# Fannovel16/ComfyUI-Frame-Interpolation

Hardware: AMD Instinct MI355X
Metric: interpolated frames/sec/GPU @1080p RIFE4.7 2x (higher is better)
Workload: dtype f32; 1 GPU; RIFE 4.7 2x, 1080x1920 synthetic frame-pair stream, 32 pairs/step/GPU resident in HBM (BASELINE.json configs[1]; SURVEY 8d config 2 clip: 33 frames torch.manual_seed(0) torch.rand); seeded random-init weights; new_frame_collective=none, launch=one process, one GPU

## Files before the change

comfyui-frame-interpolation_amd/csrc/rife_net.hip:

```cpp
#include <cmath>
#include <cstring>

#include "../../include/vfi_hip.h"
#include "../../include/vfi_hip_test.h"
#include "rife_ops.h"

using namespace vfi;

namespace {

struct DevBuf {
    float* p = nullptr;
    size_t n = 0;
    bool view = false;
    int ensure(size_t count) {
        if (count <= n) return 0;
        if (p && !view) (void)hipFree(p);
        p = nullptr;
        n = 0;
        view = false;
        VFI_CHECK_HIP(hipMalloc((void**)&p, count * sizeof(float)));
        n = count;
        return 0;
    }
// ... 33 lines not shown
    DevBuf w, ww, bias, beta;
    DevBuf bias3;
    int Cout3_p = 0;
    int Cin = 0, Cin_p = 0, Cout = 0, Cout_p = 0;
    bool folded = false;
};

const int kBlockC[5] = {192, 128, 96, 64, 32};
constexpr int kMaxBlocks = 5;

}

struct vfi_rife {
    ConvLayer conv00[kMaxBlocks], conv01[kMaxBlocks], res[kMaxBlocks][8], last[kMaxBlocks];
    DevBuf enc_w0, enc_b0, enc_w1, enc_b1;
    int arch = 47, NF = 1, CM = 16, CF = 4, n_mid = 0, nblocks = 4, NX = 0;
    bool enc_act = false;
    int last_out() const { return NX ? 52 : 24; }
    int tplanes() const { return NX ? 4 : 2; }
    DevBuf FEAT;
    ConvLayer enc_mid[2];
    DevBuf E2;
    int block_in(int i) const { return i == 0 ? 7 + 8 * NF : 12 + 8 * NF + NX; }
    int CX(int i) const { return round_up(block_in(i), 8); }
    int H = 0, W = 0, Hp = 0, Wp = 0, max_batch = 0, n_slots = 0;
    int scales[kMaxBlocks] = {8, 4, 2, 1, 1};
    int up[kMaxBlocks] = {1, 1, 1, 1, 1};
    DevBuf Ppool, E, F, F2, M, X, A0, A1, A2, T;
    DevBuf S0pool;
    std::vector<unsigned char> s0_valid;
    size_t stage0_stride() const { return (size_t)(Hp / 8) * (Wp / 8) * 8; }
    bool fused_pack() const { return n_mid == 0 && CM == 16 && CF == 4 && !enc_act && NF == 1; }
    DevBuf X1, T1;
    DevBuf Fdbg[kMaxBlocks], Xdbg[kMaxBlocks];
    bool keep = false;
    int last_B = 0;
    float* arena = nullptr;
    size_t arena_n = 0;
    std::vector<WeightView> views;
    int device = 0;
    size_t pack_stride() const { return (size_t)Hp * Wp * 4 * (1 + NF); }
};

static int bind_arena(vfi_rife* net, const std::vector<WeightView>& views, size_t n, const float* host) {
    VFI_CHECK_HIP(hipGetDevice(&net->device));
    VFI_CHECK_HIP(hipMalloc((void**)&net->arena, n * sizeof(float)));
    net->arena_n = n;
    if (host) VFI_CHECK_HIP(hipMemcpy(net->arena, host, n * sizeof(float), hipMemcpyHostToDevice));
    net->views = views;
    for (const WeightView& v : views) {
        DevBuf* b = (DevBuf*)((char*)net + v.delta);
        b->p = net->arena + v.off;
        b->n = v.count;
        b->view = true;
    }
    return 0;
}

static int make_conv3x3(ConvLayer& L, const float* w, const float* b, const float* beta, int Cout, int Cin,
                        int Cin_p, bool wino = false) {
    L.Cin = Cin;
    L.Cin_p = Cin_p;
    L.Cout = Cout;
    L.Cout_p = round_up(Cout, 32);
    std::vector<float> wp, bp;
    std::vector<float> wfold;
// ... 163 lines not shown

int vfi_rife_weights(vfi_rife_t* net, float** arena_dev, int64_t* count) {
    VFI_REQUIRE(net && net->arena && arena_dev && count, "vfi_rife_weights: null argument / no weights");
    *arena_dev = net->arena;
    *count = (int64_t)net->arena_n;
    return 0;
}

void vfi_rife_destroy(vfi_rife_t* net) {
    if (!net) return;
    for (int b = 0; b < kMaxBlocks; ++b) {
        for (ConvLayer* L : {&net->conv00[b], &net->conv01[b], &net->last[b]}) {
            L->w.release();
            L->ww.release();
            L->bias.release();
            L->beta.release();
        }
        for (int i = 0; i < 8; ++i) {
            net->res[b][i].w.release();
            net->res[b][i].ww.release();
            net->res[b][i].bias.release();
            net->res[b][i].beta.release();
        }
        net->Fdbg[b].release();
        net->Xdbg[b].release();
    }
    for (ConvLayer& L : net->enc_mid) {
        L.w.release();
        L.ww.release();
        L.bias.release();
    }
    net->E2.release();
    for (DevBuf* d : {&net->enc_w0, &net->enc_b0, &net->enc_w1, &net->enc_b1, &net->Ppool, &net->E, &net->F, &net->F2, &net->M,
                      &net->X, &net->A0, &net->A1, &net->A2, &net->T, &net->X1, &net->T1, &net->FEAT, &net->S0pool})
        d->release();
    if (net->arena) (void)hipFree(net->arena);
    delete net;
}

int vfi_rife_configure(vfi_rife_t* net, int H, int W, int max_batch, int n_slots, float scale_factor) {
    VFI_REQUIRE(net, "vfi_rife_configure: null handle");
    VFI_REQUIRE(H > 0 && W > 0 && max_batch >= 1 && max_batch <= kMaxTasks && n_slots >= 2,
                "vfi_rife_configure: bad arguments H=%d W=%d max_batch=%d (1..%d) n_slots=%d", H, W, max_batch,
                kMaxTasks, n_slots);
    const int NB = net->nblocks;
    const float base4[kMaxBlocks] = {8.f, 4.f, 2.f, 1.f, 1.f}, base5[kMaxBlocks] = {16.f, 8.f, 4.f, 2.f, 1.f};
    const float* base = NB == 5 ? base5 : base4;
    int sc[kMaxBlocks] = {1, 1, 1, 1, 1}, up[kMaxBlocks] = {1, 1, 1, 1, 1};
    for (int i = 0; i < NB; ++i) {
        const float s = base[i] / scale_factor;
        if (s >= 1.f) {
            sc[i] = (int)s;
            up[i] = 1;
            VFI_REQUIRE((float)sc[i] == s && (sc[i] == 1 || sc[i] % 2 == 0),
                        "vfi_rife_configure: scale_factor %g gives block scale %g (supported scale_factor: 0.25, 0.5, 1, 2, 4)",
                        scale_factor, s);
        } else {
            sc[i] = 1;
            up[i] = (int)(1.f / s);
            VFI_REQUIRE((up[i] == 2 || up[i] == 4) && 1.f / (float)up[i] == s && i > 0,
                        "vfi_rife_configure: scale_factor %g gives block scale %g (supported scale_factor: 0.25, 0.5, 1, 2, 4)",
                        scale_factor, s);
        }
    }
    const int Hp = round_up(H, 64), Wp = round_up(W, 64);
    for (int i = 0; i < NB; ++i) {
        VFI_REQUIRE(Hp % (4 * sc[i]) == 0 && Wp % (4 * sc[i]) == 0,
                    "vfi_rife_configure: padded size %dx%d not divisible by 4*scale %d (the reference fails here too, "
                    "SURVEY.md App. C6)", Hp, Wp, sc[i]);
        VFI_REQUIRE((double)Hp * Wp * up[i] * up[i] * net->CX(i) < 2147483647.0,
                    "vfi_rife_configure: %dx%d is too large for scale_factor %g (block input above 2^31 elements)", H, W,
                    scale_factor);
    }
    net->H = H;
    net->W = W;
    net->Hp = Hp;
    net->Wp = Wp;
    net->max_batch = max_batch;
    net->n_slots = n_slots;
    memcpy(net->scales, sc, sizeof(sc));
    memcpy(net->up, up, sizeof(up));
    const size_t full = (size_t)Hp * Wp, B = max_batch;
    size_t x = 0, a0 = 0, a1 = 0, t = 0;
    bool any_up = false;
    for (int i = 0; i < NB; ++i) {
        any_up = any_up || up[i] > 1;
        const size_t px = full / ((size_t)sc[i] * sc[i]) * ((size_t)up[i] * up[i]);
        const size_t cx = net->CX(i);
        x = std::max(x, px * cx);
        a0 = std::max(a0, px / 4 * (kBlockC[i] / 2));
        a1 = std::max(a1, px / 16 * kBlockC[i]);
        t = std::max(t, px * 4 * net->tplanes());
    }
    if (net->Ppool.ensure(net->pack_stride() * n_slots) || net->E.ensure(full / 4 * net->CM) ||
        (net->n_mid && net->E2.ensure(full / 4 * net->CM)) || net->F.ensure(B * full * 4) || net->F2.ensure(B * full * 4) ||
        net->M.ensure(B * full) || net->X.ensure(B * x) || net->A0.ensure(B * a0) || net->A1.ensure(B * a1) ||
        net->A2.ensure(B * a1) || net->T.ensure(B * t))
        return -1;
    if (any_up && (net->X1.ensure(B * full * net->CX(1)) || net->T1.ensure(B * full * 4 * net->tplanes()))) return -1;
    if (net->NX && net->FEAT.ensure(B * full * 8)) return -1;
    net->s0_valid.assign(n_slots, 0);
    if (net->fused_pack() && net->S0pool.ensure(net->stage0_stride() * n_slots)) return -1;
    return 0;
}

static void fill_args(ConvArgs& a, const ConvLayer& L, const float* in, int in_cs, float* out, int out_cs, int N,
                      int Hin, int Win, int stride) {
    memset(&a, 0, sizeof(a));
    a.in = in;
    a.w = L.w.p;
    a.bias = L.bias.p;
    a.out = out;
    a.N = N;
    a.Hin = Hin;
    a.Win = Win;
    a.in_cs = in_cs;
    a.Hout = Hin / stride;
    a.Wout = Win / stride;
    a.out_cs = out_cs;
    a.Cin_p = L.Cin_p;
    a.cin_live = L.Cin;
    a.Cout_p = L.Cout_p;
    a.Cout = L.Cout;
}

static int load_frame_impl(vfi_rife_t* net, int slot, const float* f32, const unsigned char* u8, int C, void* stream) {
    VFI_REQUIRE(net && net->Hp > 0, "vfi_rife_load_frame: network not configured");
    VFI_REQUIRE(slot >= 0 && slot < net->n_slots && C >= 3, "vfi_rife_load_frame: bad slot %d / channels %d", slot, C);
    hipStream_t st = (hipStream_t)stream;
    float* P = net->Ppool.p + (size_t)slot * net->pack_stride();
    const int Hp = net->Hp, Wp = net->Wp;
    const bool fuse_encode = option(kOptFuseEncode) != 0;
    net->s0_valid[slot] = 0;
// ... 63 lines not shown
    return 0;
}

int vfi_f32_to_u8(const float* in_dev, uint8_t* out_dev, int64_t n, void* stream) {
    VFI_REQUIRE(in_dev && out_dev && n >= 0 && ((uintptr_t)in_dev & 15) == 0 && ((uintptr_t)out_dev & 3) == 0,
                "vfi_f32_to_u8: bad arguments (in 16-byte, out 4-byte aligned)");
    return n ? f32_to_u8_launch(in_dev, out_dev, (long)n, (hipStream_t)stream) : 0;
}

int vfi_rife_interpolate(vfi_rife_t* net, int B, const int* slot0, const int* slot1, const float* timestep,
                         float* out_dev, void* stream) {
    VFI_REQUIRE(net && net->Hp > 0, "vfi_rife_interpolate: network not configured");
    VFI_REQUIRE(B >= 1 && B <= net->max_batch, "vfi_rife_interpolate: batch %d outside 1..%d", B, net->max_batch);
    hipStream_t st = (hipStream_t)stream;
    RifeTasks tasks;
    memset(&tasks, 0, sizeof(tasks));
    for (int b = 0; b < B; ++b) {
        VFI_REQUIRE(slot0[b] >= 0 && slot0[b] < net->n_slots && slot1[b] >= 0 && slot1[b] < net->n_slots,
                    "vfi_rife_interpolate: task %d uses slots %d,%d outside 0..%d", b, slot0[b], slot1[b],
                    net->n_slots - 1);
        tasks.slot0[b] = slot0[b];
        tasks.slot1[b] = slot1[b];
        tasks.t[b] = timestep[b];
    }
    const int Hp = net->Hp, Wp = net->Wp;
    static const char* kResName[kMaxBlocks] = {"resconv_c192", "resconv_c128", "resconv_c96", "resconv_c64", "resconv_c32"};
    static const char* kC00Name[kMaxBlocks] = {"conv0a_b0", "conv0a_b1", "conv0a_b2", "conv0a_b3", "conv0a_b4"};
    static const char* kC01Name[kMaxBlocks] = {"conv0b_b0", "conv0b_b1", "conv0b_b2", "conv0b_b3", "conv0b_b4"};
    static const char* kLastName[kMaxBlocks] = {"lastconv_b0", "lastconv_b1", "lastconv_b2", "lastconv_b3", "lastconv_b4"};
    const int NB = net->nblocks, TP = net->tplanes();
    const float* feat = net->NX ? net->FEAT.p : nullptr;
    bool fused_prev = false;
    const bool fuse0a_enabled = option(kOptFuse0a) != 0;
    float* Fcur = net->F.p;
    float* Falt = net->F2.p;
    bool a0_ready = false;
    for (int i = 0; i < NB; ++i) {
        const int s = net->scales[i], u = net->up[i];
        const int Hs = Hp / s * u, Ws = Wp / s * u;
        const int c = kBlockC[i];
        const int CX = net->CX(i), NF = net->NF;
        const bool x_ready = i > 0 && (fused_prev || a0_ready);
        bool staged0 = i == 0 && option(kOptStage0) != 0 && s == 8 && u == 1 && net->fused_pack() && CX == 16;
        for (int b = 0; b < B && staged0; ++b) staged0 = net->s0_valid[tasks.slot0[b]] && net->s0_valid[tasks.slot1[b]];
        if (staged0) {
            if (stage_in0_staged_launch(net->S0pool.p, net->stage0_stride(), tasks, B, net->X.p, Hp, Wp, st)) return -1;
        } else if (!x_ready &&
            stage_in_launch(net->Ppool.p, net->pack_stride(), tasks, B, Fcur, net->M.p, i > 0 ? feat : nullptr,
                            u > 1 ? net->X1.p : net->X.p, Hp, Wp, s, CX, NF, i > 0, st))
            return -1;
        if (u > 1 && planar4_up_launch(net->X1.p, net->X.p, B, Hp, Wp, u, CX,  2 + 2 * NF + net->NX / 4, st)) return -1;
        if (net->keep) {
            const size_t n = (size_t)B * Hs * Ws * CX;
            if (net->Xdbg[i].ensure(n)) return -1;
            VFI_CHECK_HIP(hipMemcpyAsync(net->Xdbg[i].p, net->X.p, n * sizeof(float), hipMemcpyDeviceToDevice, st));
        }
        ConvArgs a;
        if (!a0_ready) {
            fill_args(a, net->conv00[i], net->X.p, CX, net->A0.p, c / 2, B, Hs, Ws, 2);
            a.in_plane = Hs * Ws * 4;
            conv3x3_taps(a);
            a.act = 1;
            a.slope = 0.2f;
            if (conv_launch(a, 2, false, -1, st, kC00Name[i])) return -1;
        }
        a0_ready = false;
        fill_args(a, net->conv01[i], net->A0.p, c / 2, net->A1.p, c, B, Hs / 2, Ws / 2, 2);
        conv3x3_taps(a);
        a.act = 1;
        a.slope = 0.2f;
        if (conv_launch(a, 2, false, -1, st, kC01Name[i])) return -1;
        float* cur = net->A1.p;
        float* nxt = net->A2.p;
        for (int r = 0; r < 8; ++r) {
            fill_args(a, net->res[i][r], cur, c, nxt, c, B, Hs / 4, Ws / 4, 1);
            conv3x3_taps(a);
            a.beta = net->res[i][r].beta.p;
            a.res = net->res[i][r].folded ? nullptr : cur;
            a.res_cs = c;
            a.act = 1;
            a.slope = 0.2f;
            if (conv_wino_mode(-1) != 1 && net->res[i][r].ww.p) {
                a.w = net->res[i][r].ww.p;
                if (conv_wino_launch(a, 0, st, kResName[i])) return -1;
            } else if (conv_launch(a, 1, false, -1, st, kResName[i])) {
                return -1;
            }
            std::swap(cur, nxt);
        }
        fill_args(a, net->last[i], cur, c, net->T.p, 128, B, Hs / 4, Ws / 4, 1);
        a.out_mode = 1;
        a.out_planes = TP;
        if (option(kOptDeconvWino) && conv_wino_mode(-1) != 1 && net->last[i].ww.p && c % 8 == 0) {
            conv3x3_taps(a);
            a.w = net->last[i].ww.p;
            a.bias = net->last[i].bias3.p;
            a.Cout = 4 * net->last[i].Cout;
            a.Cout_p = net->last[i].Cout3_p;
            if (conv_wino_launch(a, 8, st, kLastName[i])) return -1;
        } else {
            deconv4x4_taps(a);
            if (conv_launch(a, 1, true, -1, st, kLastName[i])) return -1;
        }
        const float* Tsrc = net->T.p;
        if (u > 1) {
            if (t_down_launch(net->T.p, net->T1.p, B, Hp, Wp, u, TP, st)) return -1;
            Tsrc = net->T1.p;
        }
        if (i < NB - 1) {
            const int sn = net->scales[i + 1];
            const bool on_grid = u == 1 && net->up[i + 1] == 1 && s == 2 * sn;
            fused_prev = on_grid && (sn == 4 || sn == 2 || sn == 1 || (net->NX && sn == 8));
            const bool fuse0a = fuse0a_enabled && fused_prev && sn == 1 && net->NF == 1 && !net->NX && !net->keep && i > 0 &&
                                net->CX(i + 1) == 24 && kBlockC[i + 1] == 64 && net->conv00[i + 1].Cout_p == 32;
            if (fuse0a) {
                if (trans1_conv0a_launch(net->Ppool.p, net->pack_stride(), tasks, B, Tsrc, Fcur, Falt, net->conv00[i + 1].w.p,
                                         net->conv00[i + 1].bias.p, net->A0.p, Hp, Wp, 0.2f, st))
                    return -1;
                std::swap(Fcur, Falt);
                fused_prev = false;
                a0_ready = true;
            } else if (fused_prev) {
                if (net->NX ? stage_trans_x_launch(net->Ppool.p, net->pack_stride(), tasks, B, Tsrc, Fcur, net->X.p, Hp, Wp, s, sn,
                                                   i > 0, st)
                            : stage_trans_launch(net->Ppool.p, net->pack_stride(), tasks, B, Tsrc, Fcur, net->X.p, Hp, Wp,
                                                 s, sn, NF, i > 0, st))
                    return -1;
            } else {
                if (flow_up_launch(Tsrc, Fcur, net->M.p, B, Hp, Wp, s, TP, i > 0, st)) return -1;
                if (net->NX && feat_up_launch(Tsrc, net->FEAT.p, B, Hp, Wp, s, st)) return -1;
            }
            if (net->keep) {
                const size_t n = (size_t)B * Hp * Wp * 4;
                if (net->Fdbg[i].ensure(n)) return -1;
                VFI_CHECK_HIP(hipMemcpyAsync(net->Fdbg[i].p, Fcur, n * sizeof(float), hipMemcpyDeviceToDevice, st));
            }
        } else {
            float* fd = nullptr;
            if (net->keep) {
                const size_t n = (size_t)B * Hp * Wp * 4;
                if (net->Fdbg[i].ensure(n)) return -1;
                VFI_CHECK_HIP(hipMemsetAsync(net->Fdbg[i].p, 0, n * sizeof(float), st));
                fd = net->Fdbg[i].p;
            }
            if (final_blend_launch(net->Ppool.p, net->pack_stride(), tasks, B, Tsrc, Fcur, out_dev, fd, net->H,
                                   net->W, Hp, Wp, s, TP, st))
                return -1;
        }
    }
    net->last_B = B;
    return 0;
}

#ifdef VFI_TEST_TAPS
int vfi_rife_debug_keep(vfi_rife_t* net, int on) {
    VFI_REQUIRE(net, "null handle");
    net->keep = on != 0;
    return 0;
}

int64_t vfi_rife_debug_read(vfi_rife_t* net, int what, int stage, float* host_buf, int64_t cap) {
    if (!net) {
        set_error("null handle");
        return -1;
    }
    const float* src = nullptr;
    size_t n = 0;
    if (what == 0 && stage >= 0 && stage < net->nblocks) {
// ... 46 lines not shown
```

comfyui-frame-interpolation_amd/csrc/rife_ops.h:

```cpp
#pragma once
#include "vfi_common.h"

namespace vfi {

constexpr int kMaxTasks = 32;
struct RifeTasks {
    int slot0[kMaxTasks];
    int slot1[kMaxTasks];
    float t[kMaxTasks];
};

int warp_border_launch(const float* in, const float* flow, float* out, int N, int H, int W, int C, hipStream_t s);
int prep_frame_launch(const float* src, float* P, int H, int W, int C, int Hp, int Wp, hipStream_t s);
int encode47_fused_launch(const float* f32, const unsigned char* u8, float* P, float* S, const float* w0, const float* b0, const float* w1,
                          const float* b1, int H, int W, int C, int Hp, int Wp, hipStream_t s);
int encode47_batch_launch(int n, const void* const* srcs, bool u8, float* const* packs, float* const* stages, const float* w0, const float* b0,
                          const float* w1, const float* b1, int H, int W, int C, int Hp, int Wp, hipStream_t s);
int stage_in0_staged_launch(const float* Spool, size_t stage_stride, const RifeTasks& tasks, int B, float* X, int Hp, int Wp, hipStream_t st);
int prep_frame_u8_launch(const unsigned char* src, float* P, int H, int W, int C, int Hp, int Wp, hipStream_t s);
int f32_to_u8_launch(const float* in, unsigned char* out, long n, hipStream_t s);
int encode_conv_launch(const float* P, float* E, const float* w0, const float* b0, int CM, bool act, int Hp, int Wp,
                       hipStream_t s);
int encode_deconv_launch(const float* E, float* P, const float* w1, const float* b1, int CM, int CF, int Hp, int Wp,
                         hipStream_t s);
int stage_in_launch(const float* Ppool, size_t pack_stride, const RifeTasks& tasks, int B, const float* F,
                    const float* M, const float* FEAT, float* X, int Hp, int Wp, int s, int CX, int NF, bool has_flow,
                    hipStream_t st);
int flow_up_launch(const float* T, float* F, float* M, int B, int Hp, int Wp, int s, int tp, bool has_prev, hipStream_t st);
int feat_up_launch(const float* T, float* FEAT, int B, int Hp, int Wp, int s, hipStream_t st);
int stage_trans_launch(const float* Ppool, size_t pack_stride, const RifeTasks& tasks, int B, const float* T, float* F,
                       float* X, int Hp, int Wp, int s_prev, int s_next, int NF, bool has_prev, hipStream_t st);
int trans1_conv0a_launch(const float* Ppool, size_t pack_stride, const RifeTasks& tasks, int B, const float* T, const float* Fin,
                         float* Fout, const float* wpk, const float* bias, float* A0, int Hp, int Wp, float slope, hipStream_t st);
int stage_trans_x_launch(const float* Ppool, size_t pack_stride, const RifeTasks& tasks, int B, const float* T, float* F,
                         float* X, int Hp, int Wp, int s_prev, int s_next, bool has_prev, hipStream_t st);
int final_blend_launch(const float* Ppool, size_t pack_stride, const RifeTasks& tasks, int B, const float* T,
                       const float* F, float* out, float* Fdbg, int H, int W, int Hp, int Wp, int s, int tp, hipStream_t st);
int planar4_up_launch(const float* X1, float* X, int B, int Hp, int Wp, int u, int CX, int flow_plane, hipStream_t st);
int t_down_launch(const float* T, float* T1, int B, int Hp, int Wp, int u, int tp, hipStream_t st);
int t_to_nhwc_launch(const float* T, float* out, int N, int Hq, int Wq, int C4, hipStream_t st);

}
```

comfyui-frame-interpolation_amd/csrc/rife_ops.hip:

```cpp
#include "rife_ops.h"

#include <algorithm>
#include <type_traits>
#include <atomic>
#include "rife_warp.h"
#include <cstdlib>

namespace vfi {

__device__ static inline float4 lerp4(const float4 a, const float4 b, const float4 c, const float4 d,
                                      const Tap4& t) {
    float4 r;
    r.x = a.x * t.nw + b.x * t.ne + c.x * t.sw + d.x * t.se;
    r.y = a.y * t.nw + b.y * t.ne + c.y * t.sw + d.y * t.se;
    r.z = a.z * t.nw + b.z * t.ne + c.z * t.sw + d.z * t.se;
    r.w = a.w * t.nw + b.w * t.ne + c.w * t.sw + d.w * t.se;
    return r;
}

template <int NHI>
__device__ static inline void sample_pack(const float* __restrict__ P, size_t hi_off, const Tap4& t, float4& lo,
                                          float4* hi) {
    const float4* q = (const float4*)P;
    lo = lerp4(q[t.o00], q[t.o01], q[t.o10], q[t.o11], t);
// ... 860 lines not shown
}
template <int NX, bool FULL>
__device__ static inline void tq_read(const float* __restrict__ Tb, int Hs, int Ws, int Yt, int Xt, float* v) {
    const size_t p = (size_t)Yt * Ws + Xt, ps = (size_t)Hs * Ws;
    const float4 f = ((const float4*)Tb)[p];
    v[0] = f.x; v[1] = f.y; v[2] = f.z; v[3] = f.w;
    if constexpr (FULL) {
        if constexpr (NX == 0) {
            v[4] = Tb[(ps + p) * 4];
        } else {
            const float4 p1 = ((const float4*)Tb)[ps + p], p2 = ((const float4*)Tb)[2 * ps + p];
            v[4] = p1.x; v[5] = p1.y; v[6] = p1.z; v[7] = p1.w;
            v[8] = p2.x; v[9] = p2.y; v[10] = p2.z; v[11] = p2.w;
            v[4 + NX] = Tb[(3 * ps + p) * 4];
        }
    }
}
template <int NX, bool FULL>
__device__ static inline void t_upsample_quad(const float* __restrict__ Tb, int Hi, int Wi, float rs, int Y, int X, int ql,
                                              float* out) {
    constexpr int N = FULL ? 5 + NX : 4;
    const Bil by = bil_index(Y, rs, Hi), bx = bil_index(X, rs, Wi);
    float mine[5 + NX];
    tq_read<NX, FULL>(Tb, Hi, Wi, (ql >> 1) ? by.i1 : by.i0, (ql & 1) ? bx.i1 : bx.i0, mine);
    const float wy0 = by.w0, wy1 = by.w1, wx0 = bx.w0, wx1 = bx.w1;
#pragma unroll
    for (int j = 0; j < N; ++j) {
        const float a = quad_f<0x00>(mine[j]), bb = quad_f<0x55>(mine[j]), c = quad_f<0xAA>(mine[j]), d = quad_f<0xFF>(mine[j]);
        out[j] = __fadd_rn(__fmul_rn(wy0, __fadd_rn(__fmul_rn(wx0, a), __fmul_rn(wx1, bb))),
                           __fmul_rn(wy1, __fadd_rn(__fmul_rn(wx0, c), __fmul_rn(wx1, d))));
    }
}

template <int SP, bool HAS_PREV, int NF, int NX>
__global__ __launch_bounds__(256) void stage_trans_quad_kernel(const float* __restrict__ Ppool, size_t pack_stride,
                                                               RifeTasks tasks, const float* __restrict__ T,
                                                               float* __restrict__ F, float* __restrict__ Xo, int Hp,
                                                               int Wp, int tiles_x, int xcd_per, int n_tiles) {
    static_assert(SP == 2 || SP == 4 || SP == 8, "quad transition: block scales 4->2, 8->4, 16->8");
    const int bid = xcd_per > 0 ? ((int)blockIdx.x & 7) * xcd_per + ((int)blockIdx.x >> 3) : (int)blockIdx.x;
    if (bid >= n_tiles || (xcd_per > 0 && ((int)blockIdx.x >> 3) >= xcd_per)) return;
    static_assert(NX == 0 || (NX == 8 && NF == 1), "carried block features: arch 4.26 only");
    constexpr int SI = 2 * SP;
    constexpr int OFF = SP / 2 - 1;
    constexpr int NV = 5 + NX;
    const int Hs = Hp / SP, Ws = Wp / SP, Hi = Hp / SI, Wi = Wp / SI;
    const int b = blockIdx.y;
    const int tile_y = bid / tiles_x, tile_x = bid - tile_y * tiles_x;
    const int lane = threadIdx.x & 63, wave = threadIdx.x >> 6, ql = lane & 3;
    const float* Tb = T + (size_t)b * Hi * Wi * (NX ? 16 : 8);
    const float rs = 1.0f / (float)SI, fs = (float)SI;
    const int xl = tile_x * 16 + (lane >> 2), yl = tile_y * 4 + wave;
    const int X = xl * SP + OFF + (ql & 1), Y = yl * SP + OFF + (ql >> 1);
    const bool cell_ok = xl < Ws && yl < Hs;
    float v[NV];
    if constexpr (SP == 2) {
        if (!cell_ok) return;
        t_upsample_quad<NX, true>(Tb, Hi, Wi, rs, Y, X, ql, v);
        const size_t pb = (size_t)b * Hp * Wp + (size_t)Y * Wp + X;
        float4 f = make_float4(v[0] * fs, v[1] * fs, v[2] * fs, v[3] * fs);
        if (HAS_PREV) {
            const float4 o = ((const float4*)F)[pb];
            f = make_float4(o.x + f.x, o.y + f.y, o.z + f.z, o.w + f.w);
        }
        ((float4*)F)[pb] = f;
        v[0] = f.x; v[1] = f.y; v[2] = f.z; v[3] = f.w;
    } else {
        __shared__ float centre[NV][256];
#pragma unroll
        for (int p = 0; p < SP; ++p) {
            constexpr int NH = SP / 4;
#pragma unroll
            for (int h = 0; h < NH; ++h) {
                const int col = h * 64 + lane;
                const int Yp = yl * SP + p, Xp = tile_x * 16 * SP + col;
                if (Xp < Wp && Yp < Hp) {
                    const bool crow = p == OFF || p == OFF + 1;
                    float u[NV];
                    if (crow) t_upsample_quad<NX, true>(Tb, Hi, Wi, rs, Yp, Xp, ql, u);
                    else t_upsample_quad<NX, false>(Tb, Hi, Wi, rs, Yp, Xp, ql, u);
                    const size_t pb = (size_t)b * Hp * Wp + (size_t)Yp * Wp + Xp;
                    float4 fp = make_float4(u[0] * fs, u[1] * fs, u[2] * fs, u[3] * fs);
                    if (HAS_PREV) {
                        const float4 o = ((const float4*)F)[pb];
                        fp = make_float4(o.x + fp.x, o.y + fp.y, o.z + fp.z, o.w + fp.w);
                    }
                    ((float4*)F)[pb] = fp;
                    const int ix = col & (SP - 1);
                    if (crow && (ix == OFF || ix == OFF + 1)) {
                        const int dst = wave * 64 + (col / SP) * 4 + (ix - OFF) + ((p - OFF) << 1);
                        centre[0][dst] = fp.x; centre[1][dst] = fp.y; centre[2][dst] = fp.z; centre[3][dst] = fp.w;
#pragma unroll
                        for (int j = 4; j < NV; ++j) centre[j][dst] = u[j];
                    }
                }
            }
        }
        __syncthreads();
// ... 13 lines not shown
        const Tap4 t1 = warp_taps(g, X, Y, v[2], v[3]);
        float4 a_lo, b_lo, a_hi[NF], b_hi[NF];
        sample_pack<NF>(P0, hi_off, t0, a_lo, a_hi);
        sample_pack<NF>(P1, hi_off, t1, b_lo, b_hi);
        cat_inputs<NF>(r, a_lo, b_lo, a_hi, b_hi, tasks.t[b]);
#pragma unroll
        for (int j = 4; j < NV; ++j) r[3 + 8 * NF + j] = v[j];
        r[NC - 4] = v[0]; r[NC - 3] = v[1]; r[NC - 2] = v[2]; r[NC - 1] = v[3];
    }
#pragma unroll
    for (int c = 0; c < NC; ++c) {
        const float row = __fadd_rn(0.5f * r[c], 0.5f * quad_f<0xB1>(r[c]));
        r[c] = __fadd_rn(0.5f * row, 0.5f * quad_f<0x4E>(row));
    }
#pragma unroll
    for (int c = NC; c < NR; ++c) r[c] = 0.f;
    const float inv_s = 1.0f / (float)SP;
#pragma unroll
    for (int c = NC - 4; c < NC; ++c) r[c] = r[c] * inv_s;
    float4* op = (float4*)Xo + (size_t)b * (NR / 4) * Hs * Ws + (size_t)yl * Ws + xl;
#pragma unroll
    for (int base = 0; base < NR / 4; base += 4) {
        float4 val = make_float4(r[4 * base], r[4 * base + 1], r[4 * base + 2], r[4 * base + 3]);
#pragma unroll
        for (int j = 1; j < 4; ++j)
            if (base + j < NR / 4 && ql == j)
                val = make_float4(r[4 * (base + j)], r[4 * (base + j) + 1], r[4 * (base + j) + 2], r[4 * (base + j) + 3]);
        if (base + ql < NR / 4) op[(size_t)(base + ql) * Hs * Ws] = val;
    }
}

static int stage_quad_mask() { return (int)option(kOptStageQuad); }

int stage_trans_launch(const float* Ppool, size_t pack_stride, const RifeTasks& tasks, int B, const float* T, float* F,
                       float* X, int Hp, int Wp, int s_prev, int s_next, int NF, bool has_prev, hipStream_t st) {
    VFI_REQUIRE(s_prev == 2 * s_next && (s_next == 4 || s_next == 2 || s_next == 1) && (NF == 1 || NF == 2),
                "stage_trans: scales %d -> %d (%d feature planes) not on the fused path", s_prev, s_next, NF);
    const int Hs = Hp / s_next, Ws = Wp / s_next;
    const int tiles_x = cdiv(Ws, 16), tiles_y = cdiv(Hs, 16);
    dim3 grid(tiles_x * tiles_y, B);
    TraceScope ts(s_next == 4 ? "stage_trans4" : (s_next == 2 ? "stage_trans2" : "stage_trans1"), st);
    if ((s_next == 2 || s_next == 4) && (stage_quad_mask() & s_next)) {
        const int qtx = cdiv(Ws, 16);
        const int q_tiles = qtx * cdiv(Hs, 4);
        const int q_per = option(kOptXcdBands) ? cdiv(q_tiles, 8) : 0;
        dim3 qgrid(q_per ? q_per * 8 : q_tiles, B);
#define VFI_SQ(SPV, HP, NFV) \
    hipLaunchKernelGGL((stage_trans_quad_kernel<SPV, HP, NFV, 0>), qgrid, dim3(256), 0, st, Ppool, pack_stride, tasks, T, F, X, Hp, Wp, qtx, q_per, q_tiles)
#define VFI_SQ2(SPV, HP) \
    do { if (NF == 1) VFI_SQ(SPV, HP, 1); else VFI_SQ(SPV, HP, 2); } while (0)
        if (s_next == 4) {
            if (has_prev) VFI_SQ2(4, true); else VFI_SQ2(4, false);
        } else {
            if (has_prev) VFI_SQ2(2, true); else VFI_SQ2(2, false);
        }
#undef VFI_SQ2
#undef VFI_SQ
        VFI_CHECK_HIP(hipGetLastError());
        return 0;
    }
#define VFI_ST(SPV, HP, NFV) \
    hipLaunchKernelGGL((stage_trans_kernel<SPV, HP, NFV>), grid, dim3(256), 0, st, Ppool, pack_stride, tasks, T, F, X, Hp, Wp, tiles_x)
#define VFI_ST2(SPV, HP) \
    do { if (NF == 1) VFI_ST(SPV, HP, 1); else VFI_ST(SPV, HP, 2); } while (0)
    if (s_next == 4) {
        if (has_prev) VFI_ST2(4, true); else VFI_ST2(4, false);
    } else if (s_next == 2) {
        if (has_prev) VFI_ST2(2, true); else VFI_ST2(2, false);
    } else {
        if (has_prev) VFI_ST2(1, true); else VFI_ST2(1, false);
    }
#undef VFI_ST2
#undef VFI_ST
    VFI_CHECK_HIP(hipGetLastError());
    return 0;
}

constexpr int F0_TWO = 16, F0_THO = 8;
constexpr int F0_TWI = 2 * F0_TWO + 1, F0_THI = 2 * F0_THO + 1;
constexpr int F0_NPIX = F0_TWI * F0_THI;
constexpr int F0_S = 20;
constexpr int F0_XF = F0_NPIX * F0_S;
constexpr int F0_WF = 27 * 32 * 8;
constexpr int F0_THREADS = 512;
typedef float f32x16_t __attribute__((ext_vector_type(16)));
typedef float f32x4_t __attribute__((ext_vector_type(4)));

// ... 265 lines not shown
        o[15] = m;
#pragma unroll
        for (int j = 0; j < 8; ++j) o[16 + j] = gg[j];
        o[24] = f.x; o[25] = f.y; o[26] = f.z; o[27] = f.w;
#pragma unroll
        for (int c = 0; c < NC; ++c) row[c] = dx == 0 ? o[c] : __fadd_rn(0.5f * row[c], 0.5f * o[c]);
        if (dx == NP - 1) {
#pragma unroll
            for (int c = 0; c < NC; ++c) r[c] = dy == 0 ? row[c] : __fadd_rn(0.5f * r[c], 0.5f * row[c]);
        }
    }
    const float inv_s = 1.0f / (float)SP;
#pragma unroll
    for (int c = NC - 4; c < NC; ++c) r[c] = r[c] * inv_s;
    float4* op = (float4*)Xo + (size_t)b * (NR / 4) * Hs * Ws + (size_t)yl * Ws + xl;
#pragma unroll
    for (int q = 0; q < NR / 4; ++q) op[(size_t)q * Hs * Ws] = make_float4(r[4 * q], r[4 * q + 1], r[4 * q + 2], r[4 * q + 3]);
}

int stage_trans_x_launch(const float* Ppool, size_t pack_stride, const RifeTasks& tasks, int B, const float* T, float* F,
                         float* X, int Hp, int Wp, int s_prev, int s_next, bool has_prev, hipStream_t st) {
    VFI_REQUIRE(s_prev == 2 * s_next && (s_next == 8 || s_next == 4 || s_next == 2 || s_next == 1),
                "stage_trans_x: scales %d -> %d not on the fused path", s_prev, s_next);
    const int Hs = Hp / s_next, Ws = Wp / s_next;
    const int tiles_x = cdiv(Ws, 16), tiles_y = cdiv(Hs, 16);
    dim3 grid(tiles_x * tiles_y, B);
    TraceScope ts(s_next == 8 ? "stage_transx8" : (s_next == 4 ? "stage_transx4" : (s_next == 2 ? "stage_transx2" : "stage_transx1")), st);
    if (s_next >= 2 && (stage_quad_mask() & s_next)) {
        const int qtx = cdiv(Ws, 16);
        const int q_tiles = qtx * cdiv(Hs, 4);
        const int q_per = option(kOptXcdBands) ? cdiv(q_tiles, 8) : 0;
        dim3 qgrid(q_per ? q_per * 8 : q_tiles, B);
#define VFI_SQ(SPV, HP) \
    hipLaunchKernelGGL((stage_trans_quad_kernel<SPV, HP, 1, 8>), qgrid, dim3(256), 0, st, Ppool, pack_stride, tasks, T, F, X, Hp, Wp, qtx, q_per, q_tiles)
#define VFI_SQ2(SPV) \
    do { if (has_prev) VFI_SQ(SPV, true); else VFI_SQ(SPV, false); } while (0)
        if (s_next == 8) VFI_SQ2(8);
        else if (s_next == 4) VFI_SQ2(4);
        else VFI_SQ2(2);
#undef VFI_SQ2
#undef VFI_SQ
        VFI_CHECK_HIP(hipGetLastError());
        return 0;
    }
#define VFI_ST(SPV, HP) \
    hipLaunchKernelGGL((stage_trans_x_kernel<SPV, HP>), grid, dim3(256), 0, st, Ppool, pack_stride, tasks, T, F, X, Hp, Wp, tiles_x)
#define VFI_ST2(SPV) \
    do { if (has_prev) VFI_ST(SPV, true); else VFI_ST(SPV, false); } while (0)
    if (s_next == 8) VFI_ST2(8);
    else if (s_next == 4) VFI_ST2(4);
    else if (s_next == 2) VFI_ST2(2);
    else VFI_ST2(1);
#undef VFI_ST2
#undef VFI_ST
    VFI_CHECK_HIP(hipGetLastError());
    return 0;
}

__global__ void final_blend_kernel(const float* __restrict__ Ppool, size_t pack_stride, RifeTasks tasks,
                                   const float* __restrict__ T, const float* __restrict__ F, float* __restrict__ out,
                                   float* __restrict__ Fdbg, int H, int W, int Hp, int Wp, int s, int tp, int xcd_per) {
    const int seg = xcd_per > 0 ? ((int)blockIdx.x & 7) * xcd_per + ((int)blockIdx.x >> 3) : (int)blockIdx.x;
    const int idx = seg * blockDim.x + threadIdx.x;
    if (idx >= H * W || (xcd_per > 0 && ((int)blockIdx.x >> 3) >= xcd_per)) return;
    const int b = blockIdx.y;
    const int X = idx % W, Y = idx / W;
    const int Hs = Hp / s, Ws = Wp / s;
// ... 163 lines not shown
```

comfyui-frame-interpolation_amd/csrc/util.hip:

```cpp
#include "vfi_common.h"

#include <cstdarg>
#include <cstdio>
#include <cstring>
#include <atomic>
#include <chrono>
#include <cstdlib>
#include <map>
#include <mutex>
#include <string>
#include <vector>

#include "../../include/vfi_hip.h"
#include "../../include/vfi_hip_test.h"

namespace vfi {

static thread_local char g_err[1024] = "";

void set_error(const char* fmt, ...) {
    va_list ap;
    va_start(ap, fmt);
    vsnprintf(g_err, sizeof(g_err), fmt, ap);
    va_end(ap);
}
const char* get_error() { return g_err; }

static const struct { const char* name; long dflt; } kOptTable[kOptCount] = {
    {"stage_quad", 14}, {"fuse_encode", 1}, {"fuse0a", 1}, {"m2n2_px", -1}, {"grouped_variant", -1}, {"splitk", 1},
    {"splat_atomic", 0}, {"splat_spill_cap", -1}, {"wino_xcd", 1}, {"deconv_wino", 1}, {"encode_batched", 1}, {"wino_quant", 1}, {"xcd_bands", 0}, {"m2m_fused", 1}, {"m2m_side", 0}, {"film_side", 1}, {"wino_probe", 0},
    {"sepconv_split_heads", 0}, {"sepconv_planar", 1}, {"stage0", 1},
};
static std::atomic<long> g_opt[kOptCount];
static std::atomic<bool> g_opt_init{false};
static std::mutex g_opt_mu;
static std::map<std::string, int> g_variant_override;
static std::atomic<int> g_variant_override_n{0};
static void opt_init() {
    if (g_opt_init.load(std::memory_order_acquire)) return;
    std::lock_guard<std::mutex> lk(g_opt_mu);
    if (g_opt_init.load(std::memory_order_relaxed)) return;
    for (int i = 0; i < kOptCount; ++i) g_opt[i].store(kOptTable[i].dflt, std::memory_order_relaxed);
    g_opt_init.store(true, std::memory_order_release);
}
long option(Option o) {
    opt_init();
    return g_opt[o].load(std::memory_order_relaxed);
}
#ifdef VFI_TEST_TAPS
int option_set(const char* name, long value) {
    opt_init();
    for (int i = 0; i < kOptCount; ++i)
        if (name && !strcmp(name, kOptTable[i].name)) {
            g_opt[i].store(value, std::memory_order_relaxed);
            return 0;
        }
    set_error("vfi_test_set_option: unknown option '%s'", name ? name : "(null)");
    return -2;
}
#endif
int variant_override(const char* trace_name) {
    if (!trace_name || !g_variant_override_n.load(std::memory_order_acquire)) return -1;
    std::lock_guard<std::mutex> lk(g_opt_mu);
    auto it = g_variant_override.find(trace_name);
// ... 292 lines not shown
```

comfyui-frame-interpolation_amd/csrc/vfi_common.h:

```cpp
#pragma once
#include <hip/hip_runtime.h>
#include <stdint.h>
#include <string>
#include <vector>

namespace vfi {

void set_error(const char* fmt, ...);
const char* get_error();

#define VFI_CHECK_HIP(expr)                                                                   \
    do {                                                                                      \
        hipError_t _e = (expr);                                                               \
        if (_e != hipSuccess) {                                                               \
            ::vfi::set_error("%s failed: %s (%s:%d)", #expr, hipGetErrorString(_e), __FILE__, \
                             __LINE__);                                                       \
            return -1;                                                                        \
        }                                                                                     \
    } while (0)

#define VFI_REQUIRE(cond, ...)          \
    do {                                \
        if (!(cond)) {                  \
            ::vfi::set_error(__VA_ARGS__); \
// ... 11 lines not shown
    TraceScope(const char* name, hipStream_t st) : s(st), on(trace_on()) {
        if (on) trace_begin(name, s);
    }
    ~TraceScope() {
        if (on) trace_end(s);
    }
};

int clock_probe_tag(const char* name);
int clock_probe_install(unsigned long long* dev_records, int capacity);
int wino_probe_read(unsigned* out32);

enum Option {
    kOptStageQuad,
    kOptFuseEncode,
    kOptFuse0a,
    kOptM2n2Px,
    kOptGroupedVariant,
    kOptSplitK,
    kOptSplatAtomic,
    kOptSplatSpillCap,
    kOptWinoXcd,
    kOptDeconvWino,
    kOptEncodeBatched,
    kOptWinoQuant,
    kOptXcdBands,
    kOptM2mFused,
    kOptM2mSide,
    kOptFilmSide,
    kOptWinoProbe,
    kOptSepconvSplitHeads,
    kOptSepconvPlanar,
    kOptStage0,
    kOptCount
};
long option(Option o);
hipStream_t stream_apart_from(hipStream_t st);
void stream_give_back(hipStream_t side);
int option_set(const char* name, long value);
int variant_override(const char* trace_name);
enum { kConvFamilyGen1 = 1, kConvFamilyGen2 = 2, kConvFamilyWino = 3 };
void conv_record_variant(int variant);
void conv_record_launch(int family, int wino_region, int form, int store, int ks, long grid_x, long work);
int conv_record_read(int32_t* out, int cap);

int launch_cus(int device_cus);

int softsplat4_launch(const float* in, const float* flow, float* out, int N, int H, int W, hipStream_t s);

constexpr int kMaxDevices = 16;

__host__ __device__ __forceinline__ int pad_index(int i, int n, int mode) {
    if (mode == 2) i = i < 0 ? -i : (i >= n ? 2 * n - 2 - i : i);
    return min(max(i, 0), n - 1);
}

static inline int cdiv(int a, int b) { return (a + b - 1) / b; }
static inline int round_up(int a, int b) { return cdiv(a, b) * b; }

struct ConvArgs {
    const float* in;
    const float* w;
    const float* bias;
    const float* beta;
    const float* res;
    float* out;
// ... 56 lines not shown
```

Baseline: 875.1 frames/s.

## Skip writing block-0 full-res flow; recompute it from low-res output in transitions

Block 0's lastconv now writes to a small T0 buffer. The 8->4 transition no longer writes the full-resolution flow F. The 4->2 transition rebuilds block 0's flow contribution by upsampling T0 on the fly instead of reading F back. This removes a full-resolution float4 write and read of the flow per batch element, at the cost of some extra upsampling arithmetic and a new option-gated code path. The debug path recomputes the flow when intermediates are kept.

```diff
diff --git a/comfyui-frame-interpolation_amd/csrc/rife_net.hip b/comfyui-frame-interpolation_amd/csrc/rife_net.hip
--- a/comfyui-frame-interpolation_amd/csrc/rife_net.hip
+++ b/comfyui-frame-interpolation_amd/csrc/rife_net.hip
@@ -89,6 +89,8 @@
     size_t stage0_stride() const { return (size_t)(Hp / 8) * (Wp / 8) * 8; }
     bool fused_pack() const { return n_mid == 0 && CM == 16 && CF == 4 && !enc_act && NF == 1; }
     DevBuf X1, T1;
+    DevBuf T0;
+    bool flow0_shape() const { return nblocks >= 3 && scales[0] == 8 && scales[1] == 4 && scales[2] == 2 && up[0] == 1 && up[1] == 1 && up[2] == 1 && !NX && (NF == 1 || NF == 2); }
     DevBuf Fdbg[kMaxBlocks], Xdbg[kMaxBlocks];
     bool keep = false;
     int last_B = 0;
@@ -318,7 +320,7 @@
     }
     net->E2.release();
     for (DevBuf* d : {&net->enc_w0, &net->enc_b0, &net->enc_w1, &net->enc_b1, &net->Ppool, &net->E, &net->F, &net->F2, &net->M,
-                      &net->X, &net->A0, &net->A1, &net->A2, &net->T, &net->X1, &net->T1, &net->FEAT, &net->S0pool})
+                      &net->X, &net->A0, &net->A1, &net->A2, &net->T, &net->X1, &net->T1, &net->T0, &net->FEAT, &net->S0pool})
         d->release();
     if (net->arena) (void)hipFree(net->arena);
     delete net;
@@ -385,6 +387,7 @@
         return -1;
     if (any_up && (net->X1.ensure(B * full * net->CX(1)) || net->T1.ensure(B * full * 4 * net->tplanes()))) return -1;
     if (net->NX && net->FEAT.ensure(B * full * 8)) return -1;
+    if (net->flow0_shape() && net->T0.ensure(B * (full / 64) * 4 * net->tplanes())) return -1;
     net->s0_valid.assign(n_slots, 0);
     if (net->fused_pack() && net->S0pool.ensure(net->stage0_stride() * n_slots)) return -1;
     return 0;
@@ -514,6 +517,7 @@
     const float* feat = net->NX ? net->FEAT.p : nullptr;
     bool fused_prev = false;
     const bool fuse0a_enabled = option(kOptFuse0a) != 0;
+    const bool flow0 = net->flow0_shape() && stage_trans_flow0_ok();
     float* Fcur = net->F.p;
     float* Falt = net->F2.p;
     bool a0_ready = false;
@@ -570,7 +574,8 @@
             }
             std::swap(cur, nxt);
         }
-        fill_args(a, net->last[i], cur, c, net->T.p, 128, B, Hs / 4, Ws / 4, 1);
+        float* Tout = flow0 && i == 0 ? net->T0.p : net->T.p;
+        fill_args(a, net->last[i], cur, c, Tout, 128, B, Hs / 4, Ws / 4, 1);
         a.out_mode = 1;
         a.out_planes = TP;
         if (option(kOptDeconvWino) && conv_wino_mode(-1) != 1 && net->last[i].ww.p && c % 8 == 0) {
@@ -584,7 +589,7 @@
             deconv4x4_taps(a);
             if (conv_launch(a, 1, true, -1, st, kLastName[i])) return -1;
         }
-        const float* Tsrc = net->T.p;
+        const float* Tsrc = Tout;
         if (u > 1) {
             if (t_down_launch(net->T.p, net->T1.p, B, Hp, Wp, u, TP, st)) return -1;
             Tsrc = net->T1.p;
@@ -606,7 +611,7 @@
                 if (net->NX ? stage_trans_x_launch(net->Ppool.p, net->pack_stride(), tasks, B, Tsrc, Fcur, net->X.p, Hp, Wp, s, sn,
                                                    i > 0, st)
                             : stage_trans_launch(net->Ppool.p, net->pack_stride(), tasks, B, Tsrc, Fcur, net->X.p, Hp, Wp,
-                                                 s, sn, NF, i > 0, st))
+                                                 s, sn, NF, i > 0, flow0 && i < 2 ? net->T0.p : nullptr, st))
                     return -1;
             } else {
                 if (flow_up_launch(Tsrc, Fcur, net->M.p, B, Hp, Wp, s, TP, i > 0, st)) return -1;
@@ -615,7 +620,11 @@
             if (net->keep) {
                 const size_t n = (size_t)B * Hp * Wp * 4;
                 if (net->Fdbg[i].ensure(n)) return -1;
-                VFI_CHECK_HIP(hipMemcpyAsync(net->Fdbg[i].p, Fcur, n * sizeof(float), hipMemcpyDeviceToDevice, st));
+                if (flow0 && i == 0) {
+                    if (flow_up_launch(Tsrc, net->Fdbg[i].p, net->M.p, B, Hp, Wp, s, TP, false, st)) return -1;
+                } else {
+                    VFI_CHECK_HIP(hipMemcpyAsync(net->Fdbg[i].p, Fcur, n * sizeof(float), hipMemcpyDeviceToDevice, st));
+                }
             }
         } else {
             float* fd = nullptr;
diff --git a/comfyui-frame-interpolation_amd/csrc/rife_ops.h b/comfyui-frame-interpolation_amd/csrc/rife_ops.h
--- a/comfyui-frame-interpolation_amd/csrc/rife_ops.h
+++ b/comfyui-frame-interpolation_amd/csrc/rife_ops.h
@@ -28,8 +28,9 @@
                     hipStream_t st);
 int flow_up_launch(const float* T, float* F, float* M, int B, int Hp, int Wp, int s, int tp, bool has_prev, hipStream_t st);
 int feat_up_launch(const float* T, float* FEAT, int B, int Hp, int Wp, int s, hipStream_t st);
+bool stage_trans_flow0_ok();
 int stage_trans_launch(const float* Ppool, size_t pack_stride, const RifeTasks& tasks, int B, const float* T, float* F,
-                       float* X, int Hp, int Wp, int s_prev, int s_next, int NF, bool has_prev, hipStream_t st);
+                       float* X, int Hp, int Wp, int s_prev, int s_next, int NF, bool has_prev, const float* T0, hipStream_t st);
 int trans1_conv0a_launch(const float* Ppool, size_t pack_stride, const RifeTasks& tasks, int B, const float* T, const float* Fin,
                          float* Fout, const float* wpk, const float* bias, float* A0, int Hp, int Wp, float slope, hipStream_t st);
 int stage_trans_x_launch(const float* Ppool, size_t pack_stride, const RifeTasks& tasks, int B, const float* T, float* F,
diff --git a/comfyui-frame-interpolation_amd/csrc/rife_ops.hip b/comfyui-frame-interpolation_amd/csrc/rife_ops.hip
--- a/comfyui-frame-interpolation_amd/csrc/rife_ops.hip
+++ b/comfyui-frame-interpolation_amd/csrc/rife_ops.hip
@@ -916,12 +916,14 @@
     }
 }
 
-template <int SP, bool HAS_PREV, int NF, int NX>
+template <int SP, bool HAS_PREV, int NF, int NX, bool FLOW0 = false>
 __global__ __launch_bounds__(256) void stage_trans_quad_kernel(const float* __restrict__ Ppool, size_t pack_stride,
                                                                RifeTasks tasks, const float* __restrict__ T,
                                                                float* __restrict__ F, float* __restrict__ Xo, int Hp,
-                                                               int Wp, int tiles_x, int xcd_per, int n_tiles) {
+                                                               int Wp, int tiles_x, int xcd_per, int n_tiles,
+                                                               const float* __restrict__ T0) {
     static_assert(SP == 2 || SP == 4 || SP == 8, "quad transition: block scales 4->2, 8->4, 16->8");
+    static_assert(!FLOW0 || (NX == 0 && ((SP == 4 && !HAS_PREV) || (SP == 2 && HAS_PREV))), "flow0: block scales 8 -> 4 -> 2 only");
     const int bid = xcd_per > 0 ? ((int)blockIdx.x & 7) * xcd_per + ((int)blockIdx.x >> 3) : (int)blockIdx.x;
     if (bid >= n_tiles || (xcd_per > 0 && ((int)blockIdx.x >> 3) >= xcd_per)) return;
     static_assert(NX == 0 || (NX == 8 && NF == 1), "carried block features: arch 4.26 only");
@@ -938,16 +940,28 @@
     const int X = xl * SP + OFF + (ql & 1), Y = yl * SP + OFF + (ql >> 1);
     const bool cell_ok = xl < Ws && yl < Hs;
     float v[NV];
-    if constexpr (SP == 2) {
+    if constexpr (SP == 2 || FLOW0) {
         if (!cell_ok) return;
         t_upsample_quad<NX, true>(Tb, Hi, Wi, rs, Y, X, ql, v);
-        const size_t pb = (size_t)b * Hp * Wp + (size_t)Y * Wp + X;
         float4 f = make_float4(v[0] * fs, v[1] * fs, v[2] * fs, v[3] * fs);
-        if (HAS_PREV) {
-            const float4 o = ((const float4*)F)[pb];
-            f = make_float4(o.x + f.x, o.y + f.y, o.z + f.z, o.w + f.w);
-        }
-        ((float4*)F)[pb] = f;
+        if constexpr (SP == 2) {
+            const size_t pb = (size_t)b * Hp * Wp + (size_t)Y * Wp + X;
+            if (HAS_PREV) {
+                float4 o;
+                if constexpr (FLOW0) {
+                    constexpr int S0 = 2 * SI;
+                    const int H0 = Hp / S0, W0 = Wp / S0;
+                    const float fs0 = (float)S0;
+                    float p[4];
+                    t_upsample_quad<0, false>(T0 + (size_t)b * H0 * W0 * 8, H0, W0, 1.0f / fs0, Y, X, ql, p);
+                    o = make_float4(p[0] * fs0, p[1] * fs0, p[2] * fs0, p[3] * fs0);
+                } else {
+                    o = ((const float4*)F)[pb];
+                }
+                f = make_float4(o.x + f.x, o.y + f.y, o.z + f.z, o.w + f.w);
+            }
+            ((float4*)F)[pb] = f;
+        }
         v[0] = f.x; v[1] = f.y; v[2] = f.z; v[3] = f.w;
     } else {
         __shared__ float centre[NV][256];
@@ -1027,10 +1041,14 @@
 
 static int stage_quad_mask() { return (int)option(kOptStageQuad); }
 
+bool stage_trans_flow0_ok() { return option(kOptFlow0) != 0 && (stage_quad_mask() & 6) == 6; }
+
 int stage_trans_launch(const float* Ppool, size_t pack_stride, const RifeTasks& tasks, int B, const float* T, float* F,
-                       float* X, int Hp, int Wp, int s_prev, int s_next, int NF, bool has_prev, hipStream_t st) {
+                       float* X, int Hp, int Wp, int s_prev, int s_next, int NF, bool has_prev, const float* T0, hipStream_t st) {
     VFI_REQUIRE(s_prev == 2 * s_next && (s_next == 4 || s_next == 2 || s_next == 1) && (NF == 1 || NF == 2),
                 "stage_trans: scales %d -> %d (%d feature planes) not on the fused path", s_prev, s_next, NF);
+    VFI_REQUIRE(!T0 || ((stage_quad_mask() & s_next) && ((s_next == 4 && !has_prev) || (s_next == 2 && has_prev))),
+                "stage_trans: scales %d -> %d (previous flow: %d) cannot take the flow from block 0's output", s_prev, s_next, (int)has_prev);
     const int Hs = Hp / s_next, Ws = Wp / s_next;
     const int tiles_x = cdiv(Ws, 16), tiles_y = cdiv(Hs, 16);
     dim3 grid(tiles_x * tiles_y, B);
@@ -1040,14 +1058,16 @@
         const int q_tiles = qtx * cdiv(Hs, 4);
         const int q_per = option(kOptXcdBands) ? cdiv(q_tiles, 8) : 0;
         dim3 qgrid(q_per ? q_per * 8 : q_tiles, B);
-#define VFI_SQ(SPV, HP, NFV) \
-    hipLaunchKernelGGL((stage_trans_quad_kernel<SPV, HP, NFV, 0>), qgrid, dim3(256), 0, st, Ppool, pack_stride, tasks, T, F, X, Hp, Wp, qtx, q_per, q_tiles)
-#define VFI_SQ2(SPV, HP) \
-    do { if (NF == 1) VFI_SQ(SPV, HP, 1); else VFI_SQ(SPV, HP, 2); } while (0)
-        if (s_next == 4) {
-            if (has_prev) VFI_SQ2(4, true); else VFI_SQ2(4, false);
+#define VFI_SQ(SPV, HP, NFV, F0) \
+    hipLaunchKernelGGL((stage_trans_quad_kernel<SPV, HP, NFV, 0, F0>), qgrid, dim3(256), 0, st, Ppool, pack_stride, tasks, T, F, X, Hp, Wp, qtx, q_per, q_tiles, T0)
+#define VFI_SQ2(SPV, HP, F0) \
+    do { if (NF == 1) VFI_SQ(SPV, HP, 1, F0); else VFI_SQ(SPV, HP, 2, F0); } while (0)
+        if (T0) {
+            if (s_next == 4) VFI_SQ2(4, false, true); else VFI_SQ2(2, true, true);
+        } else if (s_next == 4) {
+            if (has_prev) VFI_SQ2(4, true, false); else VFI_SQ2(4, false, false);
         } else {
-            if (has_prev) VFI_SQ2(2, true); else VFI_SQ2(2, false);
+            if (has_prev) VFI_SQ2(2, true, false); else VFI_SQ2(2, false, false);
         }
 #undef VFI_SQ2
 #undef VFI_SQ
@@ -1379,7 +1399,7 @@
         const int q_per = option(kOptXcdBands) ? cdiv(q_tiles, 8) : 0;
         dim3 qgrid(q_per ? q_per * 8 : q_tiles, B);
 #define VFI_SQ(SPV, HP) \
-    hipLaunchKernelGGL((stage_trans_quad_kernel<SPV, HP, 1, 8>), qgrid, dim3(256), 0, st, Ppool, pack_stride, tasks, T, F, X, Hp, Wp, qtx, q_per, q_tiles)
+    hipLaunchKernelGGL((stage_trans_quad_kernel<SPV, HP, 1, 8>), qgrid, dim3(256), 0, st, Ppool, pack_stride, tasks, T, F, X, Hp, Wp, qtx, q_per, q_tiles, (const float*)nullptr)
 #define VFI_SQ2(SPV) \
     do { if (has_prev) VFI_SQ(SPV, true); else VFI_SQ(SPV, false); } while (0)
         if (s_next == 8) VFI_SQ2(8);
diff --git a/comfyui-frame-interpolation_amd/csrc/util.hip b/comfyui-frame-interpolation_amd/csrc/util.hip
--- a/comfyui-frame-interpolation_amd/csrc/util.hip
+++ b/comfyui-frame-interpolation_amd/csrc/util.hip
@@ -29,7 +29,7 @@
 static const struct { const char* name; long dflt; } kOptTable[kOptCount] = {
     {"stage_quad", 14}, {"fuse_encode", 1}, {"fuse0a", 1}, {"m2n2_px", -1}, {"grouped_variant", -1}, {"splitk", 1},
     {"splat_atomic", 0}, {"splat_spill_cap", -1}, {"wino_xcd", 1}, {"deconv_wino", 1}, {"encode_batched", 1}, {"wino_quant", 1}, {"xcd_bands", 0}, {"m2m_fused", 1}, {"m2m_side", 0}, {"film_side", 1}, {"wino_probe", 0},
-    {"sepconv_split_heads", 0}, {"sepconv_planar", 1}, {"stage0", 1},
+    {"sepconv_split_heads", 0}, {"sepconv_planar", 1}, {"stage0", 1}, {"flow0", 1},
 };
 static std::atomic<long> g_opt[kOptCount];
 static std::atomic<bool> g_opt_init{false};
diff --git a/comfyui-frame-interpolation_amd/csrc/vfi_common.h b/comfyui-frame-interpolation_amd/csrc/vfi_common.h
--- a/comfyui-frame-interpolation_amd/csrc/vfi_common.h
+++ b/comfyui-frame-interpolation_amd/csrc/vfi_common.h
@@ -67,6 +67,7 @@
     kOptSepconvSplitHeads,
     kOptSepconvPlanar,
     kOptStage0,
+    kOptFlow0,
     kOptCount
 };
 long option(Option o);
```

Measured after the change: 879.7 frames/s, median of 6. Within noise of the previous version (+0.5%).
